# ivanacollg/MPC_CollisionAvoidance

Hardware: AMD Instinct MI355X
Metric: batched SQP-RTI solves/sec (USV, N=40 horizon, 10 obstacles) (higher is better)
Workload: dtype f64

## Files before the change

mpc_collisionavoidance_amd/csrc/linearize.hpp:

```cpp
#pragma once
#include "lanes.hpp"
#include "params.hpp"
#include "sfor.hpp"

namespace usv {

template <class M, class = void>
struct ModelCall {
    struct Pre {};
    USV_DEV static Pre prepare(const double *) { return {}; }
    USV_DEV static void fjvp(const Pre &, const double *x, const double *U, const double *s, const double *su, double *f, double *js)
    {
        M::fjvp(x, U, s, su, f, js);
    }
};
template <class M>
struct ModelCall<M, std::void_t<typename M::Pre>> {
    using Pre = typename M::Pre;
    USV_DEV static Pre prepare(const double *x) { return M::prepare(x); }
    USV_DEV static void fjvp(const Pre &p, const double *x, const double *U, const double *s, const double *su, double *f, double *js)
    {
        M::fjvp_pre(p, x, U, s, su, f, js);
    }
};

template <class M, int KCH, bool SOFT, bool MULTI = false, int MODE = 0>
struct Linearize {
    static constexpr int NX = M::NX, NU = M::NU, NZ = NX + NU;
    using WL = WsLayout<M, KCH, SOFT>;

    USV_DEV static void run(const DevPtrs &P, long gid)
    {
        const DevSpec &S = *P.spec;
        const int lane = lanes::lane();
        const int N = lanes::uniform(S.N), K = lanes::uniform(S.K);
        const long Bp = lanes::uniform(S.Bp);
        const int k = (int)(gid / Bp);
        const long g = gid - (long)k * Bp;
        const int nB = lanes::uniform(S.B);
        const long gi = g < nB ? g : (long)nB - 1;
        const long b = P.perm ? (long)P.perm[gi] : gi;
        if constexpr (MODE == 1) {
            const long owner = P.perm_cur ? (long)P.perm_cur[gi] : gi;
            const bool ready = lanes::observe(P.epoch + b) == P.tick && lanes::observe(P.epoch + owner) == P.tick;
            if (!ready) {
                if (lane == 0) lanes::set_bits(P.redo + b * P.redo_words + (k >> 5), 1 << (k & 31));
                return;
            }
        }
        if constexpr (MODE == 2) {
            if (((P.redo[b * P.redo_words + (k >> 5)] >> (k & 31)) & 1) == 0) return;
        }
        auto ld = [](const double *q) {
            if constexpr (MODE == 1) return lanes::ld_shared(q);
            else return *q;
        };
        double *tile = P.ws + (((long)k * Bp + g) * lanes::uniform(S.npt)) * LANES + lane;
        const bool xlane = lane >= NU && lane < NZ;

        double x[NX], U[NU > 0 ? NU : 1];
        const double *xk = P.x + ((long)b * (N + 1) + k) * NX;
        sfor<0, NX>([&](auto i) { x[i] = ld(xk + i); });
        if (k < N) {
            const double *uk = P.u + ((long)b * N + k) * NU;
            sfor<0, NU>([&](auto i) { U[i] = ld(uk + i); });
        } else {
            sfor<0, NU>([&](auto i) { U[i] = 0.0; });
        }

        {
            const double *Mrow = (k < N ? S.Mc : S.Me) + lane * LANES;
            const double *yr = (k < N) ? P.yref + ((long)b * N + k) * S.ny : P.yref_e + (long)b * S.ny_e;
            const int ny = (k < N) ? S.ny : S.ny_e;
            double acc = 0.0;
            for (int y = 0; y < ny; y++) acc = fma(-Mrow[y], yr[y], acc);
            tile[WL::P_GQ * LANES] = acc;
        }
        if (k == N) return;

        const int nsteps = MULTI ? S.sim_steps : 1;
        const double dt = S.dt / (double)nsteps;
        double s0[NX], f[NX], js[NX], xs[NX], ss[NX], xa[NX], sa[NX], su[NU > 0 ? NU : 1];
        sfor<0, NU>([&](auto l) { su[l] = (lane == l) ? 1.0 : 0.0; });
        sfor<0, NX>([&](auto i) { s0[i] = (lane == NU + i) ? 1.0 : 0.0; });
        using MC = ModelCall<M>;
        const typename MC::Pre pre = MC::prepare(x);
        for (int step = 0; step < nsteps; step++) {
            MC::fjvp(pre, x, U, s0, su, f, js);
            sfor<0, NX>([&](auto i) {
                xa[i] = f[i];
                sa[i] = js[i];
                xs[i] = fma(0.5 * dt, f[i], x[i]);
                ss[i] = fma(0.5 * dt, js[i], s0[i]);
            });
            MC::fjvp(pre, xs, U, ss, su, f, js);
            sfor<0, NX>([&](auto i) {
                xa[i] = fma(2.0, f[i], xa[i]);
                sa[i] = fma(2.0, js[i], sa[i]);
                xs[i] = fma(0.5 * dt, f[i], x[i]);
                ss[i] = fma(0.5 * dt, js[i], s0[i]);
            });
            MC::fjvp(pre, xs, U, ss, su, f, js);
            sfor<0, NX>([&](auto i) {
                xa[i] = fma(2.0, f[i], xa[i]);
                sa[i] = fma(2.0, js[i], sa[i]);
                xs[i] = fma(dt, f[i], x[i]);
                ss[i] = fma(dt, js[i], s0[i]);
// ... 33 lines not shown
```

mpc_collisionavoidance_amd/csrc/params.hpp:

```cpp
#pragma once

namespace usv {

constexpr int LANES = 16;
constexpr int KMAX = 32;

struct DevSpec {
    double Hc[LANES * LANES];
    double He[LANES * LANES];
    double Mc[LANES * LANES];
    double Me[LANES * LANES];
    double lb[LANES], ub[LANES];
    int has_b[LANES];
    int boxpack;
    int boxpack_ok;
    int box_dense;
    int aux_dense4;
    int box_slot[LANES];
    int box_step[LANES];
    int slot_var[LANES];
    int slot_is[LANES];
    double uh[KMAX];
    double lsl[KMAX], lsu[KMAX];
    double zl[KMAX], zu[KMAX], Zl[KMAX], Zu[KMAX];
// ... 67 lines not shown
constexpr int wide_ex_fwd(int kch, bool softbox) { return 4 * (kch > 1 ? kch : 1) + 2 + (softbox ? 2 : 0); }
constexpr int wide_ex_planes(int kch, bool softbox = false)
{
    const int z = 4 + 2 * (kch > 1 ? kch : 1) + 1 + (softbox ? 1 : 0);
    return z > wide_ex_fwd(kch, softbox) ? z : wide_ex_fwd(kch, softbox);
}
constexpr int wide_ex_planes_hbm(int kch, bool softbox = false)
{
    const int a = 4 + 2 * (kch > 1 ? kch : 1) + 1 + (softbox ? 1 : 0) + 2;
    return a > wide_ex_fwd(kch, softbox) ? a : wide_ex_fwd(kch, softbox);
}

template <class M, int KCH, bool SOFT, bool SOFTBOX = false>
struct WsLayout {
    enum : int { P_Z = 0, P_AUX, P_DZA, P_DZ, P_DX0, P_PB, P_PI, P_BLL, P_BLU, P_BTL, P_BTU, P_OBS };
    enum : int { AXL_ZX = 15, AXL_ZY = 14, AXL_RG = 13, AXL_LU = 11, AUX_DENSE_LANES = 8 };
    static constexpr int OBSN = SOFT ? 10 : 4;
    static constexpr int P_LZU = P_OBS + KCH * OBSN;
    static constexpr int P_RB0 = P_LZU + M::NU;
    static constexpr int P_GQ = P_RB0 + 1;
    static constexpr int P_MAT = P_GQ + 1;
    static constexpr int P_BS = P_MAT + MatPack<M>::NPK;
    static constexpr int NPT = P_BS + (SOFTBOX ? 6 : 0);
};

struct DevPtrs {
    const DevSpec *spec;
    const int *perm;
    double *x;
    double *u;
    const double *x0;
    const double *yref;
    const double *yref_e;
    const double *p;
    const double *lh;
    double *sl, *su;
    double *pi;
    int *status;
    int *qp_iter;
    int *qp_status;
    double *res;
    double *obs_tmin;
    int *fail_count;
    double *nlp_res;
    int *sqp_iter;
    int *sqp_state;
    int *sqp_running;
    double *ws;
    int *queue;
    int *epoch;
    int *redo;
    int redo_words;
    const int *perm_cur;
    int tick;
    double *lam_out, *t_out;
    int nlam;
    int *susp_count;
    int *susp_list;
    double *susp_rec;
    int handover_iter;
    int *co_ctl;
};

}
```

mpc_collisionavoidance_amd/csrc/usvmpc.hip:

```cpp
#ifndef USV_PART
#define USV_PART -1
#endif
#define USV_MAIN (USV_PART <= 0)

#include "gfx950/lanes.hpp"

#include "guidance.hpp"
#include "host_spec.hpp"
#include "linearize.hpp"
#include "models.hpp"
#include "qp_ipm.hpp"
#include "sim.hpp"
#include "cond_launch.hpp"
#ifdef USV_GEN_MODEL_HEADER
#include USV_GEN_MODEL_HEADER
#endif

#include <algorithm>
#include <cstdint>
#include <cstdio>
#include <cstring>
#include <mutex>
#include <string>
#include <unordered_map>
#include <vector>

using namespace usv;

#ifndef USV_LIN_BLOCKS
#define USV_LIN_BLOCKS 2
#endif
template <class M, int KCH, bool SOFT, bool MULTI, int MODE = 0>
__global__ void __launch_bounds__(256, USV_LIN_BLOCKS) usv_linearize(DevPtrs P, long ngroups)
{
    const long gid = lanes::group_linear();
    if (gid >= ngroups) return;
    Linearize<M, KCH, SOFT, MULTI, MODE>::run(P, gid);
}

#ifndef USV_QP_WAVES
#define USV_QP_WAVES 2
#endif
template <int KCH, bool SOFTBOX>
constexpr int qp_waves() { return (KCH >= 2 || SOFTBOX) ? 1 : USV_QP_WAVES; }

template <class M, int KCH, bool SOFT, bool HDIAG, bool PACK, bool SOFTBOX, bool LDSWS = false, bool MERGE = false, bool AUXLDS = false, bool WIDE = false,
          int WW = 1, bool CPC = true>
__global__ void __launch_bounds__(64 * WW, ((LDSWS || WIDE) ? 1 : qp_waves<KCH, SOFTBOX>())) usv_qp_rti(DevPtrs P, long ngroups, int phase, int queue0, int rows)
{
    const int row = (int)(threadIdx.x >> 4);
    const long g0 = (long)blockIdx.x * rows;
    if (g0 >= ngroups) return;
    if constexpr (!WIDE && !LDSWS) { if (P.co_ctl != nullptr && threadIdx.x == 0) lanes::count_one(P.co_ctl + 2); }
    const bool has = row < rows;
    QpIpm<M, KCH, SOFT, HDIAG, PACK, SOFTBOX, LDSWS, MERGE, AUXLDS, WIDE, WW, CPC> q(P, has ? g0 + row : g0, has ? row : -1);
    q.solve(phase, queue0);
}
template <class M, int KCH, bool SOFT, bool MERGE, bool LDSWS = true, int WW = 1, bool SOFTBOX = false, bool UNPACKED = false>
constexpr auto wide_kernel()
{
    if constexpr (SOFTBOX || (UNPACKED && KCH > 0)) {
        if constexpr (WW == 1 && !MERGE) return &usv_qp_rti<M, KCH, SOFT, true, false, SOFTBOX, LDSWS, false, false, true, 1>;
        else return (decltype(&usv_qp_rti<M, KCH, SOFT, true, false, SOFTBOX, true, false>))nullptr;
    } else if constexpr (KCH == 1 || KCH == 2) return &usv_qp_rti<M, KCH, SOFT, true, true, false, LDSWS, MERGE, false, true, WW>;
    else if constexpr (KCH == 0 && !MERGE) return &usv_qp_rti<M, KCH, SOFT, true, false, false, LDSWS, false, false, true, WW>;
    else return (decltype(&usv_qp_rti<M, KCH, SOFT, true, (KCH > 0), false, true, MERGE>))nullptr;
}
template <class M, int KCH, bool SOFT, bool MERGE, bool LDSWS>
__global__ void __launch_bounds__(64, 1) usv_qp_resume(DevPtrs P)
{
    const int n = lanes::uniform(*P.susp_count);
    const bool co = P.co_ctl != nullptr;
    for (int i = (int)blockIdx.x; i < n; i += (int)gridDim.x) {
        int g = P.susp_list[i];
        if (co) {
            if (threadIdx.x == 0) g = (g >= 0 && lanes::claim(P.susp_list + i, g)) ? g : -1;
            g = lanes::wave_first_i(g);
            if (g < 0) continue;
        }
        QpIpm<M, KCH, SOFT, true, (KCH > 0), false, LDSWS, MERGE, false, true, 1> q(P, (long)g, (threadIdx.x >> 4) == 0 ? 0 : -1);
        q.solve(3, -1);
    }
}
template <class M, int KCH, bool SOFT, bool MERGE>
__global__ void __launch_bounds__(64, 1) usv_qp_resume_co(DevPtrs P, int main_wgs, int cap, int spin_limit)
{
    int *ctl = P.co_ctl;
    {
        int ok = 0;
        if (threadIdx.x == 0) ok = lanes::observe(ctl + 2) >= main_wgs;
// ... 2 lines not shown
    for (;;) {
        int t = 0;
        if (threadIdx.x == 0) t = atomicAdd(ctl, 1);
        t = lanes::wave_first_i(t);
        if (t >= cap) return;
        int e, spins = 0;
        for (;;) {
            e = lanes::observe(P.susp_list + t);
            if (e != -1) break;
            if (lanes::observe(ctl + 1) != 0) { e = lanes::observe(P.susp_list + t); break; }
            if (++spins > spin_limit) break;
            __builtin_amdgcn_s_sleep(64);
        }
        e = lanes::wave_first_i(e);
        if (e == -1) {
            if (spins > spin_limit && threadIdx.x == 0) lanes::count_one(ctl + 4);
            return;
        }
        int mine = 0;
        if (threadIdx.x == 0) mine = (e >= 0 && lanes::claim(P.susp_list + t, e)) ? 1 : 0;
        if (!lanes::wave_first_i(mine)) continue;
        lanes::acquire_agent();
        {
            QpIpm<M, KCH, SOFT, true, (KCH > 0), false, true, MERGE, false, true, 1> q(P, (long)e, (threadIdx.x >> 4) == 0 ? 0 : -1);
            q.solve(3, -1);
        }
        if (threadIdx.x == 0) lanes::count_one(ctl + 3);
    }
}
static __global__ void usv_co_done(int *ctl) { lanes::publish(ctl + 1, 1); }
using qp_resume_t = void (*)(DevPtrs);
using qp_resume_co_t = void (*)(DevPtrs, int, int, int);
template <class M, int KCH, bool SOFT, bool MERGE, bool LDSWS = false>
constexpr qp_resume_t resume_kernel()
{
    if constexpr (KCH == 1 || (KCH == 0 && !MERGE)) return &usv_qp_resume<M, KCH, SOFT, MERGE, LDSWS>;
    else return nullptr;
}
template <class M, int KCH, bool SOFT, bool MERGE>
constexpr qp_resume_co_t resume_co_kernel()
{
    if constexpr (KCH == 1 || (KCH == 0 && !MERGE)) return &usv_qp_resume_co<M, KCH, SOFT, MERGE>;
    else return nullptr;
}
using qp_kernel_t = void (*)(DevPtrs, long, int, int, int);
using group_kernel_t = void (*)(DevPtrs, long);

struct Kernels {
    qp_kernel_t qp, qp_lds, qp_aux;
    qp_kernel_t wide_lds1, wide_hbm1, wide_lds4, wide_hbm4;
    qp_resume_t resume, resume_lds;
    qp_resume_co_t resume_co;
    int nplw, ex_lds, ex_hbm;
    group_kernel_t lin[2][3];
    group_kernel_t qp_export;
    int npt_hard, npt_soft;
    int kch;
    bool soft;
};

template <class M, int KCH, bool SOFT, bool MERGE, bool SOFTBOX = false, bool UNPACKED = false>
void set_wide(Kernels &k)
{
    using WL = WsLayout<M, KCH, SOFT, SOFTBOX>;
    constexpr bool packed = KCH > 0 && !SOFTBOX && !UNPACKED;
    constexpr bool resumes = !(SOFTBOX || (UNPACKED && KCH > 0));
    k.wide_lds1 = wide_kernel<M, KCH, SOFT, MERGE, true, 1, SOFTBOX, UNPACKED>();
    k.wide_hbm1 = wide_kernel<M, KCH, SOFT, MERGE, false, 1, SOFTBOX, UNPACKED>();
    k.wide_lds4 = wide_kernel<M, KCH, SOFT, MERGE, true, 4, SOFTBOX, UNPACKED>();
    k.wide_hbm4 = wide_kernel<M, KCH, SOFT, MERGE, false, 4, SOFTBOX, UNPACKED>();
    k.resume = resumes ? resume_kernel<M, KCH, SOFT, MERGE>() : nullptr;
    k.resume_lds = resumes ? resume_kernel<M, KCH, SOFT, MERGE, true>() : nullptr;
    k.resume_co = resumes ? resume_co_kernel<M, KCH, SOFT, MERGE>() : nullptr;
    k.nplw = WL::P_RB0 - (packed ? 4 : 0) + (SOFTBOX ? 6 : 0);
    k.ex_lds = wide_ex_planes(KCH, SOFTBOX);
    k.ex_hbm = wide_ex_planes_hbm(KCH, SOFTBOX);
}

template <class M, int KCH, bool SOFT, bool PACK, bool SOFTBOX>
__global__ void __launch_bounds__(64) usv_qp_export(DevPtrs P, long ngroups)
{
    const long g0 = (long)blockIdx.x * 4;
    if (g0 >= ngroups) return;
    QpIpm<M, KCH, SOFT, true, PACK, SOFTBOX> q(P, g0 + (long)(threadIdx.x >> 4));
    q.export_rows();
}

static __global__ void __launch_bounds__(256) usv_count_unconverged(const int *qp_status, int B, int *count, unsigned long long *total)
{
    __shared__ int loc;
    if (threadIdx.x == 0) loc = 0;
    __syncthreads();
    const int i = blockIdx.x * blockDim.x + threadIdx.x;
    if (i < B && qp_status[i] != 0) atomicAdd(&loc, 1);
    __syncthreads();
    if (threadIdx.x == 0 && loc != 0) { atomicAdd(count, loc); atomicAdd(total, (unsigned long long)loc); }
}

#if USV_MAIN
__global__ void usv_sqp_begin(DevPtrs P, int B)
{
    const int i = blockIdx.x * blockDim.x + threadIdx.x;
    if (i < B) { P.sqp_state[i] = -1; P.sqp_iter[i] = 0; }
}
__global__ void usv_sqp_end(DevPtrs P, int B)
{
    const int i = blockIdx.x * blockDim.x + threadIdx.x;
// ... 74 lines not shown
}

__global__ void usv_debug_obstacle(int n, int K, const double *pos, const double *p, double *h, double *grad)
{
    const int i = blockIdx.x * blockDim.x + threadIdx.x;
    if (i >= n * K) return;
    const int pt = i / K, k = i - pt * K;
    double d, ux, uy;
    usv::obs_dist(pos[2 * pt] - p[(long)pt * 2 * K + 2 * k], pos[2 * pt + 1] - p[(long)pt * 2 * K + 2 * k + 1], d, ux, uy);
    h[i] = d; grad[2 * i] = ux; grad[2 * i + 1] = uy;
}

__global__ void __launch_bounds__(64) usv_calib_stream(DevPtrs P, long ngroups, int nread)
{
    const long g = lanes::group_linear();
    if (g >= ngroups) return;
    const lanes::Planes W(P.ws, (unsigned)(ngroups * (nread + 1) * 128), lanes::Planes::lane_offset(g, nread + 1, lanes::lane()));
    double acc = 0.0;
    for (int i = 0; i < nread; i++) acc += W.ld(i);
    W.st(nread, acc);
}
#endif

constexpr int SORT_BINS = 64;

__device__ __forceinline__ int sort_key(const int *qp_iter, const int *qp_iter_prev, int i)
{
    return min(max(max(qp_iter[i], qp_iter_prev[i]), 0), SORT_BINS - 1);
}

static __global__ void __launch_bounds__(256) usv_sort_hist(const int *qp_iter, const int *qp_iter_prev, int B, int *hist)
{
    __shared__ int loc[SORT_BINS];
    if (threadIdx.x < SORT_BINS) loc[threadIdx.x] = 0;
    __syncthreads();
    const int i = blockIdx.x * blockDim.x + threadIdx.x;
    if (i < B) atomicAdd(&loc[sort_key(qp_iter, qp_iter_prev, i)], 1);
    __syncthreads();
    if (threadIdx.x < SORT_BINS && loc[threadIdx.x] != 0) atomicAdd(&hist[threadIdx.x], loc[threadIdx.x]);
}

static __global__ void usv_sort_scan(int *hist, int *cursor)
{
    if (threadIdx.x == 0) {
        int pos = 0;
        for (int b = SORT_BINS - 1; b >= 0; b--) {
            cursor[b] = pos;
            pos += hist[b];
            hist[b] = 0;
        }
    }
}

static __global__ void __launch_bounds__(256) usv_sort_scatter(const int *qp_iter, const int *qp_iter_prev, int B, int *cursor, int *perm)
{
    __shared__ int loc[SORT_BINS], base[SORT_BINS];
    if (threadIdx.x < SORT_BINS) loc[threadIdx.x] = 0;
    __syncthreads();
    const int i = blockIdx.x * blockDim.x + threadIdx.x;
    int bin = 0, rank = 0;
    if (i < B) {
        bin = sort_key(qp_iter, qp_iter_prev, i);
        rank = atomicAdd(&loc[bin], 1);
    }
    __syncthreads();
    if (threadIdx.x < SORT_BINS && loc[threadIdx.x] != 0) base[threadIdx.x] = atomicAdd(&cursor[threadIdx.x], loc[threadIdx.x]);
    __syncthreads();
    if (i < B) perm[base[bin] + rank] = i;
}

struct usvmpc_handle {
    usvmpc_desc desc;
    DevSpec spec;
    DevPtrs ptrs;
    int nx, nu, nz, ny, ny_e, N, K, B, Bp, kch;
    bool soft;
    int device;
    hipStream_t stream;
    bool own_stream;
    static constexpr int RING = 64;
    hipEvent_t ev[RING][4];
    long nsolves;
    DevSpec *d_spec;
    int *d_perm, *d_hist, *d_cursor, *d_iter_prev;
    GuidancePtrs gd;
    bool gd_ready;
    int gd_npts_cap;
    double *gd_psi;
    double *gd_world;
    size_t gd_world_cap;
    bool sort_enabled;
    bool sort_two;
    bool merge_rows;
    bool dynamic_rows;
    int lds_mode;
    long lds_cap;
    int wide_mode;
    long wide_cap;
    long wide_hbm_cap;
    int wide_waves;
    long wide4_cap, wide4_hbm_cap;
    int last_wide;
    int handover_iter;
    int *d_susp_count, *d_susp_list;
    double *d_susp_rec;
    long resume_cap;
    int handover_co;
    int co_spin_limit;
    long co_wgs;
    bool co_ready;
    hipStream_t co_stream;
    hipEvent_t ev_co_pre, ev_co_end;
    int *d_co_ctl;
    bool ev3_set[RING];
    bool resume_lds, handover_lds;
    long max_waves;
    int ncu;
    long qp_cap;
    bool aux_lds;
    long aux_cap;
    bool map_changed;
    unsigned noise_mask;
    long long instance_offset;
    int *d_fail_ring;
    int *d_unconv_ring;
    unsigned long long *d_unconv_total;
    enum { F_X = 0, F_U, F_STATUS, F_X0, F_YREF, F_YREF_E, F_P, F_LH, F_COUNT };
    char *arena;
    char *mirror;
    size_t arena_bytes, f_off[F_COUNT + 1], f_len[F_COUNT];
    size_t dirty_lo[F_COUNT], dirty_hi[F_COUNT];
    std::vector<char> dirty_stage[F_COUNT];
    bool inflight;
    bool out_valid;
    bool extern_access;
    bool pipeline;
    hipStream_t aux_stream;
    hipEvent_t ev_pre, ev_spec;
    int *d_epoch, *d_redo, *d_perm2;
    long spec_for;
    bool spec_valid;
    bool spec_outstanding;
    int spec_quiet;
    long spec_hits, spec_misses;
    const int *spec_perm;
    int cond_N2;
    CondDims cond_dims;
    CondDims *d_cond_dims;
    double *d_cond_scratch;
    long cond_teams;
    size_t cond_lds;
    long export_at;
    bool last_cond;
    bool layout_dirty;
    size_t bytes;
    std::string err;
    std::vector<void *> allocs;
};

template <class M, int KCH, bool SOFT>
Kernels kernels_for(const usvmpc_handle *h)
{
    constexpr bool CANPACK = KCH > 0;
    const DevSpec &S = h->spec;
    const bool pack = CANPACK && S.boxpack != 0;
    Kernels k = {};
    k.lin[0][0] = &usv_linearize<M, KCH, SOFT, false, 0>; k.lin[0][1] = &usv_linearize<M, KCH, SOFT, false, 1>; k.lin[0][2] = &usv_linearize<M, KCH, SOFT, false, 2>;
    k.lin[1][0] = &usv_linearize<M, KCH, SOFT, true, 0>; k.lin[1][1] = &usv_linearize<M, KCH, SOFT, true, 1>; k.lin[1][2] = &usv_linearize<M, KCH, SOFT, true, 2>;
    k.qp_export = S.any_bsoft ? &usv_qp_export<M, KCH, SOFT, false, true>
                              : pack ? &usv_qp_export<M, KCH, SOFT, CANPACK, false> : &usv_qp_export<M, KCH, SOFT, false, false>;
    k.npt_hard = WsLayout<M, KCH, SOFT, false>::NPT; k.npt_soft = WsLayout<M, KCH, SOFT, true>::NPT;
    k.kch = KCH; k.soft = SOFT;
    auto qp = [&k](qp_kernel_t q, qp_kernel_t q_lds = nullptr, qp_kernel_t q_aux = nullptr) { k.qp = q; k.qp_lds = q_lds; k.qp_aux = q_aux; };
    const bool merge = pack && h->merge_rows && !S.box_dense;
#ifdef USV_BENCH_ONLY
    if (!(S.hdiag && pack && !S.any_bsoft)) return k;
    if (merge) {
        qp(&usv_qp_rti<M, KCH, SOFT, true, CANPACK, false, false, CANPACK>, &usv_qp_rti<M, KCH, SOFT, true, CANPACK, false, true, CANPACK>,
           &usv_qp_rti<M, KCH, SOFT, true, CANPACK, false, false, CANPACK, true>);
        set_wide<M, KCH, SOFT, CANPACK>(k);
    } else {
        qp(&usv_qp_rti<M, KCH, SOFT, true, CANPACK, false>, &usv_qp_rti<M, KCH, SOFT, true, CANPACK, false, true>,
           &usv_qp_rti<M, KCH, SOFT, true, CANPACK, false, false, false, true>);
    }
#else
    if (S.any_bsoft) {
        if (S.hdiag) { qp(&usv_qp_rti<M, KCH, SOFT, true, false, true>); set_wide<M, KCH, SOFT, false, true>(k); }
        else qp(&usv_qp_rti<M, KCH, SOFT, false, false, true>);
    } else if (S.hdiag) {
        if (merge) {
            qp(&usv_qp_rti<M, KCH, SOFT, true, CANPACK, false, false, CANPACK>, &usv_qp_rti<M, KCH, SOFT, true, CANPACK, false, true, CANPACK>,
               &usv_qp_rti<M, KCH, SOFT, true, CANPACK, false, false, CANPACK, true>);
            set_wide<M, KCH, SOFT, CANPACK>(k);
        } else if (pack) {
            qp(&usv_qp_rti<M, KCH, SOFT, true, CANPACK, false>, &usv_qp_rti<M, KCH, SOFT, true, CANPACK, false, true>,
               &usv_qp_rti<M, KCH, SOFT, true, CANPACK, false, false, false, true>);
            set_wide<M, KCH, SOFT, false>(k);
        } else {
            qp(&usv_qp_rti<M, KCH, SOFT, true, false, false>, &usv_qp_rti<M, KCH, SOFT, true, false, false, true>);
            set_wide<M, KCH, SOFT, false, false, true>(k);
        }
    } else {
        qp(pack ? &usv_qp_rti<M, KCH, SOFT, false, CANPACK, false> : &usv_qp_rti<M, KCH, SOFT, false, false, false>);
    }
#endif
    return k;
}

template <int PART> struct PartPair;
#define USV_KERNELS(PART, M, KCH, SOFT)                                                              \
    template <> struct PartPair<PART> { using Model = M; static constexpr int kch = KCH; static constexpr bool soft = SOFT; }; \
    extern template Kernels kernels_for<M, KCH, SOFT>(const usvmpc_handle *);
#if USV_PART >= 0 && !defined(USV_GEN_ONLY)
USV_KERNELS(1, ModelM0, 0, false)
USV_KERNELS(2, ModelM1, 1, true)
USV_KERNELS(3, ModelM1, 2, true)
USV_KERNELS(4, ModelM2, 1, false)
USV_KERNELS(5, ModelM2, 2, false)
#if USV_PART > 0
template Kernels kernels_for<PartPair<USV_PART>::Model, PartPair<USV_PART>::kch, PartPair<USV_PART>::soft>(const usvmpc_handle *);
#endif
// ... 451 lines not shown
            const int nb = nb_lds > 0 ? nb_lds : blocks_per_cu(k.resume, qp_block, xbytes);
            h->resume_lds = nb_lds > 0;
            h->resume_cap = (nb > 0 && h->ncu > 0) ? (long)std::min(nb, 4) * h->ncu : -1;
        }
        if (h->resume_lds) { kern_resume = k.resume_lds; xbytes = lbytes; }
        if (h->resume_cap > 0 && !h->d_susp_list) {
            if (dev_alloc(h, &h->d_susp_count, (size_t)usvmpc_handle::RING, true) || dev_alloc(h, &h->d_susp_list, (size_t)h->B, false) ||
                dev_alloc(h, &h->d_susp_rec, (size_t)h->B * 4, false))
                return USVMPC_E_HIP;
        }
        const bool small = h->qp_cap > 0 && (long)h->B <= 3 * h->qp_cap;
        hand_it = h->handover_iter > 0 ? h->handover_iter : ((h->resume_lds && small) ? 20 : 0);
        hand = h->resume_cap > 0 && hand_it > 0;
    }
    h->ptrs.susp_count = hand ? h->d_susp_count + h->nsolves % usvmpc_handle::RING : nullptr;
    h->ptrs.susp_list = hand ? h->d_susp_list : nullptr;
    h->ptrs.susp_rec = hand ? h->d_susp_rec : nullptr;
    h->ptrs.handover_iter = hand ? hand_it : 0;
    const dim3 qg((unsigned)((ng * LANES + qp_block - 1) / qp_block)), qb(qp_block);
    const bool co = hand && h->handover_co != 0 && h->resume_lds && k.resume_co != nullptr && h->own_stream && co_prepare(h);
    if (co) {
        HIP_TRY(h, set_dynamic_lds((const void *)k.resume_co, xbytes));
        h->ptrs.co_ctl = h->d_co_ctl + 8 * (h->nsolves % usvmpc_handle::RING);
        HIP_TRY(h, hipMemsetAsync(h->ptrs.co_ctl, 0, 8 * sizeof(int), h->stream));
        HIP_TRY(h, hipMemsetAsync(h->d_susp_list, 0xff, (size_t)h->B * sizeof(int), h->stream));
        HIP_TRY(h, hipEventRecord(h->ev_co_pre, h->stream));
    }
    hipLaunchKernelGGL(kern, qg, qb, aux_bytes, h->stream, h->ptrs, ng, phase, q0, 4);
    if (co) {
        hipLaunchKernelGGL(usv_co_done, dim3(1), dim3(1), 0, h->stream, h->ptrs.co_ctl);
        HIP_TRY(h, hipStreamWaitEvent(h->co_stream, h->ev_co_pre, 0));
        long nco = std::min<long>(h->resume_cap, (long)h->B);
        nco = std::min<long>(nco, h->co_wgs > 0 ? (long)h->co_wgs : (long)std::max(h->ncu, 1));
        hipLaunchKernelGGL(k.resume_co, dim3((unsigned)nco), dim3(qp_block), xbytes, h->co_stream, h->ptrs, (int)qg.x, (int)h->B, h->co_spin_limit);
        HIP_TRY(h, hipEventRecord(h->ev_co_end, h->co_stream));
    }
    if (hand) {
        HIP_TRY(h, hipEventRecord(ev[3], h->stream));
        h->ev3_set[h->nsolves % usvmpc_handle::RING] = true;
        const long nwg = std::min<long>(h->resume_cap, (long)h->B);
        hipLaunchKernelGGL(kern_resume, dim3((unsigned)nwg), dim3(qp_block), xbytes, h->stream, h->ptrs);
    }
    if (co) HIP_TRY(h, hipStreamWaitEvent(h->stream, h->ev_co_end, 0));
    return 0;
}

int launch_solve(usvmpc_handle *h, const Kernels &k, int phase)
{
    {
        const int rcf = mirror_flush(h);
        if (rcf) return rcf;
    }
    const long lin_groups = (long)(h->N + 1) * h->Bp;
    const int lin_block = 256;
    const long lin_grid = (lin_groups * LANES + lin_block - 1) / lin_block;
    hipEvent_t *ev = h->ev[h->nsolves % usvmpc_handle::RING];
    const int B = h->B;
    auto sort_into = [&](int *dst) {
        const int *prev2 = h->sort_two ? h->d_iter_prev : h->ptrs.qp_iter;
        hipLaunchKernelGGL(usv_sort_hist, dim3((B + 255) / 256), dim3(256), 0, h->stream, h->ptrs.qp_iter, prev2, B, h->d_hist);
        hipLaunchKernelGGL(usv_sort_scan, dim3(1), dim3(64), 0, h->stream, h->d_hist, h->d_cursor);
        hipLaunchKernelGGL(usv_sort_scatter, dim3((B + 255) / 256), dim3(256), 0, h->stream, h->ptrs.qp_iter, prev2, B, h->d_cursor, dst);
    };
    const group_kernel_t *lin = k.lin[h->spec.sim_steps > 1 ? 1 : 0];
    const bool cond = phase == 0 && h->cond_N2 > 0;
    const bool pipe = phase == 0 && h->pipeline && !h->mirror && !h->extern_access && h->dynamic_rows && h->B >= 16384 && !cond;
    if (pipe && !h->aux_stream) {
        int prio_least = 0, prio_greatest = 0;
        HIP_TRY(h, hipDeviceGetStreamPriorityRange(&prio_least, &prio_greatest));
        HIP_TRY(h, hipStreamCreateWithPriority(&h->aux_stream, hipStreamNonBlocking, prio_least));
        HIP_TRY(h, hipEventCreateWithFlags(&h->ev_pre, hipEventDisableTiming));
        HIP_TRY(h, hipEventCreateWithFlags(&h->ev_spec, hipEventDisableTiming));
        if (dev_alloc(h, &h->d_epoch, (size_t)B, false) || dev_alloc(h, &h->d_redo, (size_t)B * ((h->N + 32) / 32), true) ||
            dev_alloc(h, &h->d_perm2, (size_t)B, true))
            return USVMPC_E_HIP;
        HIP_TRY(h, hipMemsetAsync(h->d_epoch, 0xff, (size_t)B * sizeof(int), h->stream));
    }
    if (h->spec_outstanding) {
        HIP_TRY(h, hipStreamWaitEvent(h->stream, h->ev_spec, 0));
        h->spec_outstanding = false;
    }
    const bool had_spec = pipe && h->spec_for == h->nsolves;
    const bool use_spec = had_spec && h->spec_valid;
    if (had_spec) (use_spec ? h->spec_hits : h->spec_misses)++;
    h->spec_valid = false;
    if (use_spec) {
        h->ptrs.perm = h->spec_perm;
        h->map_changed = true;
    } else if (h->sort_enabled && h->nsolves > 0 && phase != 2) {
        if (phase == 0) h->map_changed = true;
        sort_into(h->d_perm);
        HIP_TRY(h, hipGetLastError());
        h->ptrs.perm = h->d_perm;
    }
    constexpr int SPEC_QUIET_MIN = 2;
    if (pipe) h->spec_quiet++;
    const bool spec_next = pipe && h->spec_quiet >= SPEC_QUIET_MIN;
    h->ptrs.epoch = spec_next ? h->d_epoch : nullptr;
    h->ptrs.redo = pipe ? h->d_redo : nullptr;
    h->ptrs.redo_words = (h->N + 32) / 32;
    h->ptrs.perm_cur = nullptr;
    h->ptrs.tick = (int)h->nsolves;
    h->ev3_set[h->nsolves % usvmpc_handle::RING] = false;
    HIP_TRY(h, hipEventRecord(ev[0], h->stream));
    hipLaunchKernelGGL(lin[use_spec ? 2 : 0], dim3((unsigned)lin_grid), dim3(lin_block), 0, h->stream, h->ptrs, lin_groups);
    HIP_TRY(h, hipGetLastError());
    if (pipe) HIP_TRY(h, hipMemsetAsync(h->d_redo, 0, (size_t)B * ((h->N + 32) / 32) * sizeof(int), h->stream));
    HIP_TRY(h, hipEventRecord(ev[1], h->stream));
    h->ptrs.fail_count = h->d_fail_ring + h->nsolves % usvmpc_handle::RING;
    HIP_TRY(h, hipMemsetAsync(h->ptrs.fail_count, 0, sizeof(int), h->stream));
    HIP_TRY(h, hipMemsetAsync(h->d_unconv_ring + h->nsolves % usvmpc_handle::RING, 0, sizeof(int), h->stream));
    if (h->d_susp_count) HIP_TRY(h, hipMemsetAsync(h->d_susp_count + h->nsolves % usvmpc_handle::RING, 0, sizeof(int), h->stream));
    const int *next_perm = nullptr;
    if (spec_next) {
        if (h->sort_enabled) {
            int *dst = (h->ptrs.perm == h->d_perm) ? h->d_perm2 : h->d_perm;
            sort_into(dst);
            HIP_TRY(h, hipGetLastError());
            next_perm = dst;
        }
        HIP_TRY(h, hipEventRecord(h->ev_pre, h->stream));
    }
    if (h->sort_enabled && h->sort_two && phase == 0)
        HIP_TRY(h, hipMemcpyAsync(h->d_iter_prev, h->ptrs.qp_iter, (size_t)h->B * sizeof(int), hipMemcpyDeviceToDevice, h->stream));
    if (h->spec.npt != (h->spec.any_bsoft ? k.npt_soft : k.npt_hard)) {
        h->err = "workspace layout mismatch between host and kernels";
        return USVMPC_E_ARG;
    }
    if (!cond && k.qp == nullptr) { h->err = "development build: bench instantiation only"; return USVMPC_E_ARG; }
    const int rcq = cond ? launch_cond(h) : launch_qp(h, k, phase);
    if (rcq) return rcq;
    HIP_TRY(h, hipGetLastError());
    HIP_TRY(h, hipEventRecord(ev[2], h->stream));
    if (phase == 0) {
        hipLaunchKernelGGL(usv_count_unconverged, dim3((B + 255) / 256), dim3(256), 0, h->stream, h->ptrs.qp_status, B,
                           h->d_unconv_ring + h->nsolves % usvmpc_handle::RING, h->d_unconv_total);
        HIP_TRY(h, hipGetLastError());
    }
    if (spec_next) {
        HIP_TRY(h, hipStreamWaitEvent(h->aux_stream, h->ev_pre, 0));
        DevPtrs Pn = h->ptrs;
        Pn.perm = next_perm;
        Pn.perm_cur = h->ptrs.perm;
        hipLaunchKernelGGL(lin[1], dim3((unsigned)lin_grid), dim3(lin_block), 0, h->aux_stream, Pn, lin_groups);
        HIP_TRY(h, hipGetLastError());
        HIP_TRY(h, hipEventRecord(h->ev_spec, h->aux_stream));
        h->spec_for = h->nsolves + 1;
        h->spec_valid = true;
        h->spec_outstanding = true;
        h->spec_perm = next_perm;
    }
    h->nsolves++;
    h->layout_dirty = false;
    h->last_cond = cond;
    if (h->mirror) {
        HIP_TRY(h, hipMemcpyAsync(h->mirror, h->arena, h->f_off[usvmpc_handle::F_X0], hipMemcpyDeviceToHost, h->stream));
        h->inflight = true;
        h->out_valid = true;
    }
    return 0;
}

int model_mat_planes(int model)
{
    switch (model) {
#ifndef USV_GEN_ONLY
    case USVMPC_MODEL_USV: return MatPack<ModelM0>::NPK;
    case USVMPC_MODEL_GUIDANCE_CA1: return MatPack<ModelM1>::NPK;
    case USVMPC_MODEL_PF_CA: return MatPack<ModelM2>::NPK;
#endif
#ifdef USV_GEN_MODEL_HEADER
    case USVMPC_MODEL_GENERATED: return MatPack<ModelGen>::NPK;
#endif
    }
    return 0;
}

bool model_kernels(const usvmpc_handle *h, Kernels &k)
{
    switch (h->desc.model) {
#ifdef USV_BENCH_ONLY
    case USVMPC_MODEL_PF_CA: if (h->kch <= 1) { k = kernels_for<ModelM2, 1, false>(h); return true; } break;
    case USVMPC_MODEL_GUIDANCE_CA1: if (h->kch <= 1) { k = kernels_for<ModelM1, 1, true>(h); return true; } break;
#elif !defined(USV_GEN_ONLY)
    case USVMPC_MODEL_USV: k = kernels_for<ModelM0, 0, false>(h); return true;
    case USVMPC_MODEL_GUIDANCE_CA1: k = h->kch <= 1 ? kernels_for<ModelM1, 1, true>(h) : kernels_for<ModelM1, 2, true>(h); return true;
    case USVMPC_MODEL_PF_CA: k = h->kch <= 1 ? kernels_for<ModelM2, 1, false>(h) : kernels_for<ModelM2, 2, false>(h); return true;
#endif
#if defined(USV_GEN_MODEL_HEADER) && !defined(USV_BENCH_ONLY)
    case USVMPC_MODEL_GENERATED: k = kernels_for<ModelGen, USV_GEN_KCH, (USV_GEN_SOFT != 0)>(h); return true;
#endif
    }
    return false;
}

int launch(usvmpc_handle *h, int phase = 0)
{
// ... 120 lines not shown
int usvmpc_create(const usvmpc_desc *d, usvmpc_handle **out)
{
    if (!d || !out) return USVMPC_E_ARG;
    *out = nullptr;
    DevSpec S;
    const std::string err = build_spec(*d, S);
    if (!err.empty()) {
        g_create_err = err;
        std::fprintf(stderr, "usvmpc_create: %s\n", err.c_str());
        return USVMPC_E_ARG;
    }
    if (d->model != USVMPC_MODEL_GENERATED && (d->model == USVMPC_MODEL_GUIDANCE_CA1) != (d->soft != 0) && d->K > 0) {
        std::fprintf(stderr, "usvmpc_create: obstacle rows are soft for model 1 and hard for model 2\n");
        return USVMPC_E_ARG;
    }
#ifdef USV_GEN_MODEL_HEADER
    if (d->model == USVMPC_MODEL_GENERATED &&
        ((S.K + LANES - 1) / LANES != USV_GEN_KCH || (S.K > 0 && (d->soft != 0) != (USV_GEN_SOFT != 0)))) {
        std::fprintf(stderr, "usvmpc_create: this library was generated for %d obstacle chunk(s), soft = %d\n", USV_GEN_KCH, USV_GEN_SOFT);
        return USVMPC_E_ARG;
    }
#endif
#ifdef USV_GEN_ONLY
    if (d->model != USVMPC_MODEL_GENERATED) {
        std::fprintf(stderr, "usvmpc_create: this library only holds the generated model\n");
        return USVMPC_E_ARG;
    }
#endif
    int ndev = 0;
    if (hipGetDeviceCount(&ndev) != hipSuccess || ndev < 1 || d->device < 0 || d->device >= ndev) {
        std::fprintf(stderr, "usvmpc_create: no usable HIP device (count %d, requested %d); there is no CPU fallback\n",
                     ndev, d->device);
        return USVMPC_E_NODEVICE;
    }
    usvmpc_handle *h = new usvmpc_handle();
    h->desc = *d;
    h->spec = S;
    model_dims(d->model, h->nx, h->nu);
    h->nz = h->nx + h->nu; h->ny = S.ny; h->ny_e = S.ny_e;
    h->N = S.N; h->K = S.K; h->B = S.B; h->Bp = S.Bp;
    h->kch = d->model == USVMPC_MODEL_USV ? 0 : ((S.K + LANES - 1) / LANES > 1 ? 2 : 1);
    h->soft = d->soft != 0 || d->model == USVMPC_MODEL_GUIDANCE_CA1;
#ifdef USV_GEN_MODEL_HEADER
    if (d->model == USVMPC_MODEL_GENERATED) { h->kch = USV_GEN_KCH; h->soft = USV_GEN_SOFT != 0; }
#endif
    h->device = d->device;
    h->bytes = 0; h->nsolves = 0; h->own_stream = true;
    h->map_changed = false;
    h->export_at = -1;
    h->layout_dirty = false;
    h->last_cond = false;
    h->pipeline = true;
    h->aux_stream = nullptr; h->ev_pre = nullptr; h->ev_spec = nullptr;
    h->d_epoch = nullptr; h->d_redo = nullptr; h->d_perm2 = nullptr;
    h->spec_for = -1; h->spec_valid = false; h->spec_outstanding = false; h->spec_perm = nullptr;
    h->spec_quiet = 0; h->spec_hits = 0; h->spec_misses = 0;
    h->noise_mask = ~0u;
    h->instance_offset = 0;
    h->cond_N2 = 0; h->d_cond_dims = nullptr; h->d_cond_scratch = nullptr; h->cond_teams = 0; h->cond_lds = 0;
    h->dynamic_rows = true;
    h->qp_cap = 0;
    h->aux_lds = true;
    h->aux_cap = 0;
    h->lds_mode = -1;
    h->lds_cap = 0;
    h->wide_mode = -1; h->wide_cap = 0; h->wide_hbm_cap = 0; h->last_wide = 0;
    h->wide_waves = -1; h->wide4_cap = 0; h->wide4_hbm_cap = 0;
    h->handover_co = -1; h->co_spin_limit = 200000; h->co_wgs = 0; h->co_ready = false; h->co_stream = nullptr; h->ev_co_pre = nullptr; h->ev_co_end = nullptr; h->d_co_ctl = nullptr;
    h->handover_iter = -1; for (bool &e : h->ev3_set) e = false; h->resume_lds = false; h->handover_lds = true; h->d_susp_count = nullptr; h->d_susp_list = nullptr; h->d_susp_rec = nullptr; h->resume_cap = 0;
    h->max_waves = 0;
    {
        hipDeviceProp_t prop;
        h->ncu = (hipGetDeviceProperties(&prop, d->device) == hipSuccess) ? prop.multiProcessorCount : 0;
    }
    std::memset(&h->ptrs, 0, sizeof(h->ptrs));
    auto fail = [&](int rc) {
        std::fprintf(stderr, "usvmpc_create: %s\n", h->err.c_str());
        for (void *a : h->allocs) (void)hipFree(a);
        if (h->mirror) (void)hipHostFree(h->mirror);
        delete h;
        return rc;
    };
#define TRY_C(x) do { int rc_ = (x); if (rc_) return fail(rc_); } while (0)
#define HIP_C(call) do { hipError_t e_ = (call); if (e_ != hipSuccess) { h->err = std::string(#call) + ": " + hipGetErrorString(e_); return fail(USVMPC_E_HIP); } } while (0)
    HIP_C(hipSetDevice(h->device));
    HIP_C(hipStreamCreateWithFlags(&h->stream, hipStreamNonBlocking));
    for (int r = 0; r < usvmpc_handle::RING; r++)
        for (int i = 0; i < 4; i++) HIP_C(hipEventCreate(&h->ev[r][i]));
    const size_t B = h->B, N = h->N, K = h->K;
    const size_t stride = (size_t)h->Bp * LANES;
    const size_t kch = h->kch ? h->kch : 1;
    DevPtrs &P = h->ptrs;
    h->spec.npt = ws_planes(h->nx, h->nu, h->kch, h->soft, model_mat_planes(h->desc.model), h->spec.any_bsoft != 0);
    if ((size_t)h->Bp * (size_t)h->spec.npt * 128u > (size_t)UINT32_MAX - 16384u) {
        h->err = "batch too large for one handle: batch * " + std::to_string(h->spec.npt * 128) + " bytes per stage exceed the 4 GiB "
                 "buffer window (at most " + std::to_string((size_t)UINT32_MAX / ((size_t)h->spec.npt * 128u) / 4 * 4) + " instances); use several handles";
        return fail(USVMPC_E_ARG);
    }
    TRY_C(dev_alloc(h, &h->d_spec, 1, false));
    HIP_C(hipMemcpy(h->d_spec, &h->spec, sizeof(DevSpec), hipMemcpyHostToDevice));
    P.spec = h->d_spec;
    {
        const size_t len[usvmpc_handle::F_COUNT] = {B * (N + 1) * h->nx * sizeof(double), B * N * h->nu * sizeof(double), B * sizeof(int),
                                                    B * h->nx * sizeof(double), B * N * h->ny * sizeof(double), B * h->ny_e * sizeof(double),
                                                    B * (N + 1) * 2 * K * sizeof(double), B * N * K * sizeof(double)};
        size_t off = 0;
        for (int f = 0; f < usvmpc_handle::F_COUNT; f++) {
// ... 437 lines not shown
        break;
#endif
#ifdef USV_GEN_MODEL_HEADER
    case USVMPC_MODEL_GENERATED:
        hipLaunchKernelGGL(usv_advance_sim<ModelGen>, grid, block, 0, h->stream, h->ptrs, plant->T, plant->num_steps, sigma, seed, h->noise_mask, h->instance_offset);
        break;
#endif
    default: h->err = "advance_sim: no plant kernel for this model in this library"; return USVMPC_E_ARG;
    }
    HIP_TRY(h, hipGetLastError());
    return 0;
}

int usvmpc_set_option(usvmpc_handle *h, const char *name, double value)
{
    if (!h) return USVMPC_E_ARG;
    const std::string s(name ? name : "");
    {
        const int rcs = spec_cancel(h);
        if (rcs) return rcs;
    }
    if (s == "pipeline_linearize") { h->pipeline = value != 0.0; return 0; }
    if (s == "sort_by_difficulty") {
        h->sort_enabled = value != 0.0;
        if (!h->sort_enabled && h->ptrs.perm) { h->ptrs.perm = nullptr; h->map_changed = true; }
        return 0;
    }
    if (s == "max_waves") { h->max_waves = (long)value; reset_caps(h); cond_release(h); return 0; }
    if (s == "keep_multipliers") {
        if (value == 0.0) return 0;
        DevPtrs &P = h->ptrs;
        if (!P.lam_out) {
            HIP_TRY(h, hipSetDevice(h->device));
            P.nlam = lam_len(h->spec, h->soft);
            const size_t cnt = (size_t)h->B * (h->N + 1) * (size_t)(P.nlam > 0 ? P.nlam : 1);
            if (dev_alloc(h, &P.lam_out, cnt, false)) return USVMPC_E_HIP;
            if (dev_alloc(h, &P.t_out, cnt, false)) { P.lam_out = nullptr; return USVMPC_E_HIP; }
            h->export_at = -1;
        }
        return 0;
    }
    if (s == "qp_cond_N") {
        const int n2 = (int)value;
        if (n2 < 0 || n2 > h->N) { h->err = "qp_cond_N must lie in 0..N"; return USVMPC_E_ARG; }
        const int want = (n2 == 0 || n2 == h->N) ? 0 : n2;
        if (want > 0) {
            if (h->nx + ((h->N + want - 1) / want) * h->nu > 64) { h->err = "qp_cond_N: a condensed stage may have at most 64 variables (nx + ceil(N / qp_cond_N) nu)"; return USVMPC_E_ARG; }
            if (h->spec.any_bsoft) { h->err = "partial condensing (qp_cond_N) is not built for soft state bounds"; return USVMPC_E_ARG; }
        }
        if (want != h->cond_N2) { cond_release(h); h->cond_N2 = want; h->map_changed = true; }
        return 0;
    }
    if (s == "sort_two_ticks") { h->sort_two = value != 0.0; return 0; }
    if (s == "aux_in_lds") { h->aux_lds = value != 0.0; reset_caps(h); return 0; }
    if (s == "lds_workspace") {
        h->lds_mode = value < 0.0 ? -1 : (value > 0.0 ? 1 : 0);
        reset_caps(h);
        return 0;
    }
    if (s == "wide") {
        h->wide_mode = value < 0.0 ? -1 : (value > 0.0 ? 1 : 0);
        reset_caps(h);
        return 0;
    }
    if (s == "wide_waves") {
        h->wide_waves = value < 0.0 ? -1 : (value >= 4.0 ? 4 : 1);
        reset_caps(h);
        return 0;
    }
    if (s == "dynamic_rows") {
        h->dynamic_rows = value != 0.0;
        reset_caps(h);
        return 0;
    }
    if (s == "cond_pred_corr" || s == "cpc_factor" || s == "hpipm_mode") {
        if (s == "cpc_factor") { if (!(value > 0.0)) { h->err = "cpc_factor must be positive"; return USVMPC_E_ARG; } h->spec.cpc_factor = value; }
        else if (s == "hpipm_mode") {
            usvmpc_desc d;
            if (value != (double)(int)value || !hpipm_profile(d, (int)value)) { h->err = "hpipm_mode must be one of USVMPC_HPIPM_*"; return USVMPC_E_ARG; }
            h->spec.mu0 = d.mu0; h->spec.alpha_min = d.alpha_min; h->spec.cpc = d.cond_pred_corr; h->spec.cpc_factor = d.cpc_factor;
        } else {
            h->spec.cpc = value != 0.0 ? 1 : 0;
        }
        HIP_TRY(h, hipSetDevice(h->device));
        HIP_TRY(h, hipMemcpyAsync(h->d_spec, &h->spec, sizeof(DevSpec), hipMemcpyHostToDevice, h->stream));
        HIP_TRY(h, hipStreamSynchronize(h->stream));
        return 0;
    }
    if (s == "handover_iter") {
        if (value > 1e6) { h->err = "handover_iter out of range"; return USVMPC_E_ARG; }
        h->handover_iter = value < 0.0 ? -1 : (int)value;
        return 0;
    }
    if (s == "handover_lds") { h->handover_lds = value != 0.0; reset_caps(h); return 0; }
    if (s == "handover_co") { h->handover_co = value < 0.0 ? -1 : (value != 0.0 ? 1 : 0); return 0; }
    if (s == "handover_co_spin") { if (!(value >= 1.0 && value <= 2e9)) { h->err = "handover_co_spin out of range"; return USVMPC_E_ARG; } h->co_spin_limit = (int)value; return 0; }
    if (s == "handover_co_wgs") { if (!(value >= 0.0 && value <= 1e6)) { h->err = "handover_co_wgs out of range"; return USVMPC_E_ARG; } h->co_wgs = (long)value; return 0; }
    if (s == "disturbance_mask") {
        h->noise_mask = (unsigned)value;
        return 0;
    }
    if (s == "instance_offset") {
        if (!(value >= 0.0 && value <= 9007199254740992.0) || value != (double)(long long)value) {
            h->err = "instance_offset must be a non-negative integer";
            return USVMPC_E_ARG;
        }
// ... 381 lines not shown
```

Measured before the change: 942,100.

## Reorder speculative linearization by instance and add per-wave fixup pass

After: 960,600, median of 6. +2.0%, better.

```diff
diff --git a/mpc_collisionavoidance_amd/csrc/lin_order.hpp b/mpc_collisionavoidance_amd/csrc/lin_order.hpp
--- /dev/null
+++ b/mpc_collisionavoidance_amd/csrc/lin_order.hpp
@@ -0,0 +1,31 @@
+#pragma once
+
+#if defined(__HIPCC__) || defined(__CUDACC__)
+#define USV_HD __host__ __device__ inline
+#else
+#define USV_HD inline
+#endif
+
+namespace usv {
+
+struct LinItem {
+    long g;
+    int k;
+};
+
+USV_HD long lin_slot(long g, long B) { return g < B ? g : B - 1; }
+
+USV_HD LinItem lin_item(long item, int N, long B, const int *perm_cur, const int *inv_next)
+{
+    const long q = item / (N + 1);
+    LinItem it;
+    it.k = (int)(item - q * (N + 1));
+    it.g = q;
+    if (q < B) {
+        const long b = perm_cur ? (long)perm_cur[q] : q;
+        it.g = inv_next ? (long)inv_next[b] : b;
+    }
+    return it;
+}
+
+}
diff --git a/mpc_collisionavoidance_amd/csrc/linearize.hpp b/mpc_collisionavoidance_amd/csrc/linearize.hpp
--- a/mpc_collisionavoidance_amd/csrc/linearize.hpp
+++ b/mpc_collisionavoidance_amd/csrc/linearize.hpp
@@ -1,5 +1,6 @@
 #pragma once
 #include "lanes.hpp"
+#include "lin_order.hpp"
 #include "params.hpp"
 #include "sfor.hpp"
 
@@ -28,19 +29,41 @@
 struct Linearize {
     static constexpr int NX = M::NX, NU = M::NU, NZ = NX + NU;
     using WL = WsLayout<M, KCH, SOFT>;
+    static constexpr bool SPEC = MODE == 1 || MODE == 3, FIXUP = MODE == 2 || MODE == 4;
 
     USV_DEV static void run(const DevPtrs &P, long gid)
+    {
+        const long Bp = lanes::uniform(P.spec->Bp);
+        const int k = (int)(gid / Bp);
+        run_at(P, k, gid - (long)k * Bp);
+    }
+
+    USV_DEV static void run_item(const DevPtrs &P, long item)
+    {
+        const LinItem it = lin_item(item, P.spec->N, (long)P.spec->B, P.perm_cur, P.inv_next);
+        run_at(P, it.k, it.g);
+    }
+
+    USV_DEV static void run_marked(const DevPtrs &P, long g, int row)
+    {
+        const int N = lanes::uniform(P.spec->N);
+        const long gi = lin_slot(g, (long)lanes::uniform(P.spec->B));
+        const long b = P.perm ? (long)P.perm[gi] : gi;
+        int any = 0;
+        for (int w = 0; w < P.redo_words; w++) any |= P.redo[b * P.redo_words + w];
+        if (any == 0) return;
+        for (int k = row; k <= N; k += lanes::WAVE_ROWS) run_at(P, k, g);
+    }
+
+    USV_DEV static void run_at(const DevPtrs &P, const int k, const long g)
     {
         const DevSpec &S = *P.spec;
         const int lane = lanes::lane();
         const int N = lanes::uniform(S.N), K = lanes::uniform(S.K);
         const long Bp = lanes::uniform(S.Bp);
-        const int k = (int)(gid / Bp);
-        const long g = gid - (long)k * Bp;
-        const int nB = lanes::uniform(S.B);
-        const long gi = g < nB ? g : (long)nB - 1;
+        const long gi = lin_slot(g, (long)lanes::uniform(S.B));
         const long b = P.perm ? (long)P.perm[gi] : gi;
-        if constexpr (MODE == 1) {
+        if constexpr (SPEC) {
             const long owner = P.perm_cur ? (long)P.perm_cur[gi] : gi;
             const bool ready = lanes::observe(P.epoch + b) == P.tick && lanes::observe(P.epoch + owner) == P.tick;
             if (!ready) {
@@ -48,11 +71,11 @@
                 return;
             }
         }
-        if constexpr (MODE == 2) {
+        if constexpr (FIXUP) {
             if (((P.redo[b * P.redo_words + (k >> 5)] >> (k & 31)) & 1) == 0) return;
         }
         auto ld = [](const double *q) {
-            if constexpr (MODE == 1) return lanes::ld_shared(q);
+            if constexpr (SPEC) return lanes::ld_shared(q);
             else return *q;
         };
         double *tile = P.ws + (((long)k * Bp + g) * lanes::uniform(S.npt)) * LANES + lane;
diff --git a/mpc_collisionavoidance_amd/csrc/params.hpp b/mpc_collisionavoidance_amd/csrc/params.hpp
--- a/mpc_collisionavoidance_amd/csrc/params.hpp
+++ b/mpc_collisionavoidance_amd/csrc/params.hpp
@@ -143,6 +143,7 @@
     int *redo;
     int redo_words;
     const int *perm_cur;
+    const int *inv_next;
     int tick;
     double *lam_out, *t_out;
     int nlam;
diff --git a/mpc_collisionavoidance_amd/csrc/usvmpc.hip b/mpc_collisionavoidance_amd/csrc/usvmpc.hip
--- a/mpc_collisionavoidance_amd/csrc/usvmpc.hip
+++ b/mpc_collisionavoidance_amd/csrc/usvmpc.hip
@@ -30,12 +30,21 @@
 #ifndef USV_LIN_BLOCKS
 #define USV_LIN_BLOCKS 2
 #endif
+constexpr int LIN_MODES = 5;
+constexpr int lin_block(int mode) { return mode == 3 ? 64 : 256; }
 template <class M, int KCH, bool SOFT, bool MULTI, int MODE = 0>
-__global__ void __launch_bounds__(256, USV_LIN_BLOCKS) usv_linearize(DevPtrs P, long ngroups)
-{
-    const long gid = lanes::group_linear();
-    if (gid >= ngroups) return;
-    Linearize<M, KCH, SOFT, MULTI, MODE>::run(P, gid);
+__global__ void __launch_bounds__(lin_block(MODE), USV_LIN_BLOCKS) usv_linearize(DevPtrs P, long n)
+{
+    using L = Linearize<M, KCH, SOFT, MULTI, MODE>;
+    if constexpr (MODE == 4) {
+        const long g = (long)blockIdx.x * (lin_block(MODE) / 64) + (long)(threadIdx.x >> 6);
+        if (g < n) L::run_marked(P, g, (int)lanes::wave_row());
+    } else {
+        const long gid = lanes::group_linear();
+        if (gid >= n) return;
+        if constexpr (MODE == 3) L::run_item(P, gid);
+        else L::run(P, gid);
+    }
 }
 
 #ifndef USV_QP_WAVES
@@ -144,7 +153,7 @@
     qp_resume_t resume, resume_lds;
     qp_resume_co_t resume_co;
     int nplw, ex_lds, ex_hbm;
-    group_kernel_t lin[2][3];
+    group_kernel_t lin[2][LIN_MODES];
     group_kernel_t qp_export;
     int npt_hard, npt_soft;
     int kch;
@@ -325,7 +334,7 @@
     }
 }
 
-static __global__ void __launch_bounds__(256) usv_sort_scatter(const int *qp_iter, const int *qp_iter_prev, int B, int *cursor, int *perm)
+static __global__ void __launch_bounds__(256) usv_sort_scatter(const int *qp_iter, const int *qp_iter_prev, int B, int *cursor, int *perm, int *inv)
 {
     __shared__ int loc[SORT_BINS], base[SORT_BINS];
     if (threadIdx.x < SORT_BINS) loc[threadIdx.x] = 0;
@@ -339,7 +348,16 @@
     __syncthreads();
     if (threadIdx.x < SORT_BINS && loc[threadIdx.x] != 0) base[threadIdx.x] = atomicAdd(&cursor[threadIdx.x], loc[threadIdx.x]);
     __syncthreads();
-    if (i < B) perm[base[bin] + rank] = i;
+    if (i < B) {
+        perm[base[bin] + rank] = i;
+        if (inv) inv[i] = base[bin] + rank;
+    }
+}
+
+static __global__ void __launch_bounds__(256) usv_invert_map(const int *perm, int B, int *inv)
+{
+    const int g = blockIdx.x * blockDim.x + threadIdx.x;
+    if (g < B) inv[perm[g]] = g;
 }
 
 struct usvmpc_handle {
@@ -410,13 +428,16 @@
     bool pipeline;
     hipStream_t aux_stream;
     hipEvent_t ev_pre, ev_spec;
-    int *d_epoch, *d_redo, *d_perm2;
+    int *d_epoch, *d_redo, *d_perm2, *d_inv;
     long spec_for;
     bool spec_valid;
     bool spec_outstanding;
     int spec_quiet;
     long spec_hits, spec_misses;
     const int *spec_perm;
+    bool spec_fine;
+    int lin_force;
+    int *d_force_epoch, *d_force_redo, *d_force_inv;
     int cond_N2;
     CondDims cond_dims;
     CondDims *d_cond_dims;
@@ -439,7 +460,9 @@
     const bool pack = CANPACK && S.boxpack != 0;
     Kernels k = {};
     k.lin[0][0] = &usv_linearize<M, KCH, SOFT, false, 0>; k.lin[0][1] = &usv_linearize<M, KCH, SOFT, false, 1>; k.lin[0][2] = &usv_linearize<M, KCH, SOFT, false, 2>;
+    k.lin[0][3] = &usv_linearize<M, KCH, SOFT, false, 3>; k.lin[0][4] = &usv_linearize<M, KCH, SOFT, false, 4>;
     k.lin[1][0] = &usv_linearize<M, KCH, SOFT, true, 0>; k.lin[1][1] = &usv_linearize<M, KCH, SOFT, true, 1>; k.lin[1][2] = &usv_linearize<M, KCH, SOFT, true, 2>;
+    k.lin[1][3] = &usv_linearize<M, KCH, SOFT, true, 3>; k.lin[1][4] = &usv_linearize<M, KCH, SOFT, true, 4>;
     k.qp_export = S.any_bsoft ? &usv_qp_export<M, KCH, SOFT, false, true>
                               : pack ? &usv_qp_export<M, KCH, SOFT, CANPACK, false> : &usv_qp_export<M, KCH, SOFT, false, false>;
     k.npt_hard = WsLayout<M, KCH, SOFT, false>::NPT; k.npt_soft = WsLayout<M, KCH, SOFT, true>::NPT;
@@ -997,15 +1020,18 @@
         if (rcf) return rcf;
     }
     const long lin_groups = (long)(h->N + 1) * h->Bp;
-    const int lin_block = 256;
-    const long lin_grid = (lin_groups * LANES + lin_block - 1) / lin_block;
+    auto lin_count = [&](int mode) { return mode == 4 ? (long)h->Bp : lin_groups; };
+    auto lin_grid = [&](int mode) {
+        const long per_block = mode == 4 ? lin_block(mode) / 64 : lin_block(mode) / LANES;
+        return dim3((unsigned)((lin_count(mode) + per_block - 1) / per_block));
+    };
     hipEvent_t *ev = h->ev[h->nsolves % usvmpc_handle::RING];
     const int B = h->B;
-    auto sort_into = [&](int *dst) {
+    auto sort_into = [&](int *dst, int *inv) {
         const int *prev2 = h->sort_two ? h->d_iter_prev : h->ptrs.qp_iter;
         hipLaunchKernelGGL(usv_sort_hist, dim3((B + 255) / 256), dim3(256), 0, h->stream, h->ptrs.qp_iter, prev2, B, h->d_hist);
         hipLaunchKernelGGL(usv_sort_scan, dim3(1), dim3(64), 0, h->stream, h->d_hist, h->d_cursor);
-        hipLaunchKernelGGL(usv_sort_scatter, dim3((B + 255) / 256), dim3(256), 0, h->stream, h->ptrs.qp_iter, prev2, B, h->d_cursor, dst);
+        hipLaunchKernelGGL(usv_sort_scatter, dim3((B + 255) / 256), dim3(256), 0, h->stream, h->ptrs.qp_iter, prev2, B, h->d_cursor, dst, inv);
     };
     const group_kernel_t *lin = k.lin[h->spec.sim_steps > 1 ? 1 : 0];
     const bool cond = phase == 0 && h->cond_N2 > 0;
@@ -1017,7 +1043,7 @@
         HIP_TRY(h, hipEventCreateWithFlags(&h->ev_pre, hipEventDisableTiming));
         HIP_TRY(h, hipEventCreateWithFlags(&h->ev_spec, hipEventDisableTiming));
         if (dev_alloc(h, &h->d_epoch, (size_t)B, false) || dev_alloc(h, &h->d_redo, (size_t)B * ((h->N + 32) / 32), true) ||
-            dev_alloc(h, &h->d_perm2, (size_t)B, true))
+            dev_alloc(h, &h->d_perm2, (size_t)B, true) || dev_alloc(h, &h->d_inv, (size_t)B, true))
             return USVMPC_E_HIP;
         HIP_TRY(h, hipMemsetAsync(h->d_epoch, 0xff, (size_t)B * sizeof(int), h->stream));
     }
@@ -1034,7 +1060,7 @@
         h->map_changed = true;
     } else if (h->sort_enabled && h->nsolves > 0 && phase != 2) {
         if (phase == 0) h->map_changed = true;
-        sort_into(h->d_perm);
+        sort_into(h->d_perm, nullptr);
         HIP_TRY(h, hipGetLastError());
         h->ptrs.perm = h->d_perm;
     }
@@ -1045,10 +1071,30 @@
     h->ptrs.redo = pipe ? h->d_redo : nullptr;
     h->ptrs.redo_words = (h->N + 32) / 32;
     h->ptrs.perm_cur = nullptr;
+    h->ptrs.inv_next = nullptr;
     h->ptrs.tick = (int)h->nsolves;
     h->ev3_set[h->nsolves % usvmpc_handle::RING] = false;
     HIP_TRY(h, hipEventRecord(ev[0], h->stream));
-    hipLaunchKernelGGL(lin[use_spec ? 2 : 0], dim3((unsigned)lin_grid), dim3(lin_block), 0, h->stream, h->ptrs, lin_groups);
+    const int lin_mode = use_spec ? (h->spec_fine ? 4 : 2) : 0;
+    if (h->lin_force != 0 && lin_mode == 0 && phase == 0) {
+        const size_t nredo = (size_t)B * h->ptrs.redo_words;
+        if (!h->d_force_epoch && (dev_alloc(h, &h->d_force_epoch, (size_t)B, false) || dev_alloc(h, &h->d_force_redo, nredo, false) ||
+                                  dev_alloc(h, &h->d_force_inv, (size_t)B, false)))
+            return USVMPC_E_HIP;
+        DevPtrs Pf = h->ptrs;
+        Pf.epoch = h->d_force_epoch;
+        Pf.redo = h->d_force_redo;
+        HIP_TRY(h, hipMemsetD32Async((hipDeviceptr_t)h->d_force_epoch, h->lin_force == 1 ? Pf.tick : -1, (size_t)B, h->stream));
+        HIP_TRY(h, hipMemsetAsync(h->d_force_redo, 0, nredo * sizeof(int), h->stream));
+        if (Pf.perm) {
+            hipLaunchKernelGGL(usv_invert_map, dim3((B + 255) / 256), dim3(256), 0, h->stream, Pf.perm, B, h->d_force_inv);
+            Pf.inv_next = h->d_force_inv;
+        }
+        hipLaunchKernelGGL(lin[3], lin_grid(3), dim3(lin_block(3)), 0, h->stream, Pf, lin_count(3));
+        hipLaunchKernelGGL(lin[4], lin_grid(4), dim3(lin_block(4)), 0, h->stream, Pf, lin_count(4));
+    } else {
+        hipLaunchKernelGGL(lin[lin_mode], lin_grid(lin_mode), dim3(lin_block(lin_mode)), 0, h->stream, h->ptrs, lin_count(lin_mode));
+    }
     HIP_TRY(h, hipGetLastError());
     if (pipe) HIP_TRY(h, hipMemsetAsync(h->d_redo, 0, (size_t)B * ((h->N + 32) / 32) * sizeof(int), h->stream));
     HIP_TRY(h, hipEventRecord(ev[1], h->stream));
@@ -1060,7 +1106,7 @@
     if (spec_next) {
         if (h->sort_enabled) {
             int *dst = (h->ptrs.perm == h->d_perm) ? h->d_perm2 : h->d_perm;
-            sort_into(dst);
+            sort_into(dst, h->d_inv);
             HIP_TRY(h, hipGetLastError());
             next_perm = dst;
         }
@@ -1087,7 +1133,10 @@
         DevPtrs Pn = h->ptrs;
         Pn.perm = next_perm;
         Pn.perm_cur = h->ptrs.perm;
-        hipLaunchKernelGGL(lin[1], dim3((unsigned)lin_grid), dim3(lin_block), 0, h->aux_stream, Pn, lin_groups);
+        Pn.inv_next = next_perm ? h->d_inv : nullptr;
+        h->spec_fine = h->ptrs.susp_count == nullptr;
+        const int spec_mode = h->spec_fine ? 3 : 1;
+        hipLaunchKernelGGL(lin[spec_mode], lin_grid(spec_mode), dim3(lin_block(spec_mode)), 0, h->aux_stream, Pn, lin_count(spec_mode));
         HIP_TRY(h, hipGetLastError());
         HIP_TRY(h, hipEventRecord(h->ev_spec, h->aux_stream));
         h->spec_for = h->nsolves + 1;
@@ -1314,7 +1363,9 @@
     h->last_cond = false;
     h->pipeline = true;
     h->aux_stream = nullptr; h->ev_pre = nullptr; h->ev_spec = nullptr;
-    h->d_epoch = nullptr; h->d_redo = nullptr; h->d_perm2 = nullptr;
+    h->d_epoch = nullptr; h->d_redo = nullptr; h->d_perm2 = nullptr; h->d_inv = nullptr;
+    h->spec_fine = false;
+    h->lin_force = 0; h->d_force_epoch = nullptr; h->d_force_redo = nullptr; h->d_force_inv = nullptr;
     h->spec_for = -1; h->spec_valid = false; h->spec_outstanding = false; h->spec_perm = nullptr;
     h->spec_quiet = 0; h->spec_hits = 0; h->spec_misses = 0;
     h->noise_mask = ~0u;
@@ -1858,6 +1909,11 @@
         return 0;
     }
     if (s == "sort_two_ticks") { h->sort_two = value != 0.0; return 0; }
+    if (s == "lin_force_modes") {
+        if (value != 0.0 && value != 1.0 && value != 2.0) { h->err = "lin_force_modes: 0, 1 or 2"; return USVMPC_E_ARG; }
+        h->lin_force = (int)value;
+        return 0;
+    }
     if (s == "aux_in_lds") { h->aux_lds = value != 0.0; reset_caps(h); return 0; }
     if (s == "lds_workspace") {
         h->lds_mode = value < 0.0 ? -1 : (value > 0.0 ? 1 : 0);
```
